# nianticlabs/map-free-reloc

Measured on AMD Instinct MI355X. Metric: image-pairs/sec @ 540x720 (SuperPoint+SuperGlue + PnP w/ depth), higher is better.
Workload: dtype f32 in / f32 accumulate; matrix products of the 3x3 convolutions, attention, the transformer's linear layers and SuperPoint's 1x1 descriptor head on the f16 matrix cores with every fp32 operand carried as TWO f16 terms (xh = rne_f16(x), xl = rne_f16((x - xh) 2^11); weights pre-scaled per output feat

## Files before the change

include/mfr_hip.h:

```cpp
#ifndef MFR_HIP_H
#define MFR_HIP_H
#include <stddef.h>
#include <stdint.h>

#ifdef __cplusplus
extern "C" {
#endif

#define MFR_ABI_VERSION 6

#define MFR_K_F32 0
#define MFR_K_F64 1

#define MFR_E_ARG      (-1)
#define MFR_E_LAUNCH   (-2)
#define MFR_E_WORKSPACE (-3)

#define MFR_ST_OK          0
#define MFR_ST_TOO_FEW     1
#define MFR_ST_BAD_DEPTH   2
#define MFR_ST_NO_MODEL    3
#define MFR_ST_DEGENERATE  4

int mfr_abi_version(void);
// ... 201 lines not shown
                    long long max_record_bytes, float *gray, uint8_t *rgb, int32_t *status, int32_t *rounds, void *workspace,
                    size_t workspace_bytes, int subseq_bits, void *stream);

size_t mfr_png_depth_workspace_bytes(int n, int H, int W);
int mfr_png_depth_decode(const void *headers, const uint8_t *records, const long long *offsets, int n, int H, int W,
                         long long max_record_bytes, void *scratch, size_t scratch_bytes, float *out, int32_t *status, void *stream);

int mfr_resize_gray_bilinear(const uint8_t *rgb, int n, int H, int W, const int32_t *status,
                             const int32_t *y0, const int32_t *y1, const float *fy,
                             const int32_t *x0, const int32_t *x1, const float *fx,
                             int h, int w, float *out, void *stream);

size_t mfr_wino_f16x2_filter_bytes(int Cin, int Cout);
int mfr_wino_f16x2_filter_transform(const float *w, int Cin, int Cout, void *upk, void *stream);
int mfr_conv3x3_wino_f16x2(const float *x, const void *upk, const float *bias, const float *residual, int B, int Cin, int Cout,
                           int H, int W, int act, int pool, float *y, void *stream);
size_t mfr_conv3x3_direct_f16x2_filter_bytes(int Cin, int Cout);
int mfr_conv3x3_direct_f16x2_filter_pack(const float *w, int Cin, int Cout, void *packed, void *stream);
int mfr_conv3x3_direct_f16x2(const float *x, const void *packed, const float *bias, const float *residual, int B, int Cin, int Cout,
                             int H, int W, int act, int pool, float *y, void *stream);
int mfr_conv3x3_direct_f16x2_rows(const float *x, const void *packed, const float *bias, int B, int Cin, int Cout, int H, int W, int act, float *yrows, int ldy, void *stream);
int mfr_conv3x3_direct_f16x2_tiled(const float *x, const void *packed, const float *bias, const float *residual, int B, int Cin, int Cout, int H, int W,
                                   int act, int pool, float *y, int ldrows, int tile_mode, int pitch, void *stream);
int mfr_conv3x3s2_direct_f16x2(const float *x, const void *packed, const float *bias, int B, int Cin, int Cout, int H, int W, int act, float *y, void *stream);
int mfr_sp_conv1ab_f16x2(const float *gray, const float *w1a, const float *b1a, const void *upk1b, const float *bias1b, int B, int H, int W, float *y, void *stream);
size_t mfr_wino_bf16x3_filter_bytes(int Cin, int Cout);
int mfr_wino_bf16x3_filter_transform(const float *w, int Cin, int Cout, void *upk, void *stream);
int mfr_conv3x3_wino_bf16x3(const float *x, const void *upk, const float *bias, const float *residual, int B, int Cin, int Cout,
                            int H, int W, int act, int pool, float *y, void *stream);
size_t mfr_wino_filter_bytes(int Cin, int Cout);
int mfr_wino_filter_transform(const float *w, int Cin, int Cout, float *upk, void *stream);
int mfr_conv3x3_wino(const float *x, const float *upk, const float *bias, const float *residual, int B, int Cin, int Cout,
                     int H, int W, int act, int pool, float *y, void *stream);
int mfr_conv3x3_wino_variant(const float *x, const float *upk, const float *bias, const float *residual, int B, int Cin, int Cout,
                             int H, int W, int act, int pool, int variant, float *y, void *stream);

int mfr_corr_warp_fwd(const float *q, const float *k, const float *v, const float *grid, int B, int Dq, int N,
                      float *warped, float *pos, float *max_score, float *row_max, float *row_sum, void *stream);
int mfr_corr_warp_bwd(const float *q, const float *k, const float *v, const float *grid, int B, int Dq, int N,
                      const float *d_warped, const float *d_pos, const float *d_max, const float *delta,
                      const float *row_max, const float *row_sum, float *dq, float *dk, float *dv, void *stream);

#ifdef __cplusplus
}
#endif
#endif
// ... 1 lines not shown
```

map-free-reloc_amd/_lib.py:

```python
import ctypes as C
import os

_HERE = os.path.dirname(os.path.abspath(__file__))
SO_PATH = os.path.join(_HERE, "csrc", "libmfr_hip.so")

_lib = None

_vp, _i, _d, _u64, _sz = C.c_void_p, C.c_int, C.c_double, C.c_uint64, C.c_size_t

SIGNATURES = {
    "mfr_abi_version": (_i, []),
    "mfr_target_arch": (C.c_char_p, []),
    "mfr_f16x2_guard_bind": (_i, [_vp]),
    "mfr_test_f64_ops": (_i, [_vp, _vp, _vp, _i, _vp, _vp]),
    "mfr_test_sample": (_i, [_u64, _vp, _i, _i, _i, _i, _vp, _vp]),
    "mfr_pnp_workspace_bytes": (_sz, [_i, _i, _i]),
    "mfr_pnp_solve_batch": (_i, [_vp, _vp, _vp, _i, _i, _vp, _i, _i, _vp, _vp, _i, _i, _d, _d, _u64, _vp,
                                 _vp, _sz, _vp, _vp, _vp, _vp, _vp, _vp]),
    "mfr_depth_min": (_i, [_vp, _i, _i, _i, _vp, _vp]),
    "mfr_pnp_lift": (_i, [_vp, _vp, _vp, _i, _i, _vp, _vp, _i, _i, _vp, _i, _vp, _vp, _vp, _vp, _vp]),
    "mfr_pnp_ransac": (_i, [_vp, _vp, _vp, _i, _i, _vp, _i, _i, _d, _d, _u64, _vp, _vp, _vp, _vp, _vp, _vp, _vp,
                            _vp, _vp, _vp, _vp]),
    "mfr_emat_workspace_bytes": (_sz, [_i, _i, _i]),
    "mfr_magsac_lut": (_i, [_vp, _i]),
# ... 41 lines not shown
    "mfr_loftr_coarse_match_variant": (_i, [_vp, _i, _i, _i, _i, _i, C.c_float, C.c_float, _i, _vp, _sz, _vp, _vp, _vp, _vp, _i, _vp]),
    "mfr_loftr_fine_attention": (_i, [_vp, _i, _vp, _vp, _i, _i, _i, _i, _i, _vp, _i, _vp]),
    "mfr_loftr_gather_windows": (_i, [_vp, _i, _i, _i, _i, _vp, _vp, _i, _i, _i, _i, _vp, _vp]),
    "mfr_loftr_fine_match": (_i, [_vp, _vp, _i, _i, _i, _i, C.c_float, _vp, _vp, _vp, _vp, _vp]),
    "mfr_conv3x3_c1_relu": (_i, [_vp, _vp, _vp, _i, _i, _i, _i, _vp, _vp]),
    "mfr_bias_relu_nchw": (_i, [_vp, _vp, _i, _i, _i, _vp]),
    "mfr_conv1x1_nchw": (_i, [_vp, _vp, _vp, _i, _i, _i, _i, _vp, _vp]),
    "mfr_nchw_to_rows": (_i, [_vp, _vp, _i, _i, _i, _i, _vp, C.c_longlong, _i, _vp]),
    "mfr_nchw_to_rows_gather": (_i, [_vp, _vp, _i, _i, _i, _vp, _i, _vp, C.c_longlong, _i, _vp]),
    "mfr_bias_pool2_relu_nchw": (_i, [_vp, _vp, _i, _i, _i, _i, _vp, _vp]),
    "mfr_wino_bf16x3_filter_bytes": (_sz, [_i, _i]),
    "mfr_wino_bf16x3_filter_transform": (_i, [_vp, _i, _i, _vp, _vp]),
    "mfr_conv3x3_wino_bf16x3": (_i, [_vp, _vp, _vp, _vp, _i, _i, _i, _i, _i, _i, _i, _vp, _vp]),
    "mfr_sp_conv1ab_f16x2": (_i, [_vp, _vp, _vp, _vp, _vp, _i, _i, _i, _vp, _vp]),
    "mfr_wino_f16x2_filter_bytes": (_sz, [_i, _i]),
    "mfr_wino_f16x2_filter_transform": (_i, [_vp, _i, _i, _vp, _vp]),
    "mfr_conv3x3_wino_f16x2": (_i, [_vp, _vp, _vp, _vp, _i, _i, _i, _i, _i, _i, _i, _vp, _vp]),
    "mfr_conv3x3_direct_f16x2_filter_bytes": (_sz, [_i, _i]),
    "mfr_conv3x3_direct_f16x2_filter_pack": (_i, [_vp, _i, _i, _vp, _vp]),
    "mfr_conv3x3_direct_f16x2": (_i, [_vp, _vp, _vp, _vp, _i, _i, _i, _i, _i, _i, _i, _vp, _vp]),
    "mfr_conv3x3s2_direct_f16x2": (_i, [_vp, _vp, _vp, _i, _i, _i, _i, _i, _i, _vp, _vp]),
    "mfr_conv3x3_direct_f16x2_rows": (_i, [_vp, _vp, _vp, _i, _i, _i, _i, _i, _i, _vp, _i, _vp]),
    "mfr_conv3x3_direct_f16x2_tiled": (_i, [_vp, _vp, _vp, _vp, _i, _i, _i, _i, _i, _i, _i, _vp, _i, _i, _i, _vp]),
    "mfr_wino_filter_bytes": (_sz, [_i, _i]),
    "mfr_wino_filter_transform": (_i, [_vp, _i, _i, _vp, _vp]),
    "mfr_conv3x3_wino": (_i, [_vp, _vp, _vp, _vp, _i, _i, _i, _i, _i, _i, _i, _vp, _vp]),
    "mfr_conv3x3_wino_variant": (_i, [_vp, _vp, _vp, _vp, _i, _i, _i, _i, _i, _i, _i, _i, _vp, _vp]),
    "mfr_layernorm": (_i, [_vp, _i, _vp, _vp, _vp, _i, C.c_longlong, _i, C.c_float, _vp, _i, _vp]),
    "mfr_conv_gemm_bf16": (_i, [_vp, C.c_longlong, _vp, _vp, C.c_longlong, _vp, _i, _i, _i, _vp, _vp, C.c_longlong, _i,
                                _i, _i, _i, _vp, _vp, _vp, _vp, _vp]),
    "mfr_conv_pack_nhwc_halo": (_i, [_vp, _i, _i, _i, _i, _i, _i, _vp, _i, _vp]),
    "mfr_conv_unpack_nchw": (_i, [_vp, _i, _i, _i, _i, _i, _vp, _vp]),
    "mfr_conv_pack_cm_halo": (_i, [_vp, _i, C.c_longlong, _i, _i, _i, C.c_longlong, _i, _i, C.c_longlong, _vp, _vp]),
    "mfr_upsample2x_add": (_i, [_vp, _vp, _i, _i, _i, _vp]),
    "mfr_upsample_bilinear": (_i, [_vp, _vp, _i, _i, _i, _i, _i, _i, _vp]),
    "mfr_corr_warp_fwd": (_i, [_vp, _vp, _vp, _vp, _i, _i, _i, _vp, _vp, _vp, _vp, _vp, _vp]),
    "mfr_corr_warp_bwd": (_i, [_vp, _vp, _vp, _vp, _i, _i, _i, _vp, _vp, _vp, _vp, _vp, _vp, _vp, _vp, _vp, _vp]),
    "mfr_kabsch_fwd": (_i, [_vp, _i, _vp, _vp]),
    "mfr_kabsch_bwd": (_i, [_vp, _vp, _i, _vp, _vp]),
    "mfr_rootsift": (_i, [_vp, _i, _vp, _vp, _vp]),
    "mfr_desc_ratio_match": (_i, [_vp, _vp, _vp, _vp, _vp, _vp, _i, _i, _i, _vp, _vp, _d, _vp, _vp, _vp, _vp, _i, _vp, _vp]),
    "mfr_sift_workspace_bytes": (_sz, [_i, _i, _i, _i]),
    "mfr_sift_level_offset": (C.c_longlong, [_i, _i, _i, _i, _i, _vp, _vp]),
    "mfr_sift_blur_taps": (_i, [_i, _vp, _vp]),
    "mfr_sift_detect": (_i, [_vp, _i, _i, _i, _i, _i, _i, _vp, _sz, _vp, _vp, _vp, _vp, _vp, _vp, _vp, _vp, _vp]),
    "mfr_jpeg_workspace_bytes": (_sz, [_i, _i, _i, C.c_longlong, _i]),
# ... 57 lines not shown
```

map-free-reloc_amd/csrc/conv_direct.hip:

```cpp
#include <hip/hip_runtime.h>
#include <stdint.h>
#include <type_traits>

#include "../../include/mfr_hip.h"
#include "wave_dev.h"
#include "split_f16.h"
#include "guard.h"

using namespace mfr;

typedef float dc_f32x16 __attribute__((ext_vector_type(16)));
#define DC_OOB 0x80000000u
#define DC_PC 34
#define DC_FRAGS_PER_TAP 6
#ifndef DC_NW
#define DC_NW 4
#endif

#ifdef DC_PROF
__device__ unsigned long long dc_prof[8][64];
#define DC_STAMP(k) do { if (blockIdx.x == (gridDim.x / 2 | 5u) && lane == 0) { __builtin_amdgcn_sched_barrier(0); dc_prof[w][(k)] = __builtin_amdgcn_s_memtime(); __builtin_amdgcn_sched_barrier(0); } } while (0)
extern "C" int *mfr_guard_current(void) { return nullptr; }
#else
#define DC_STAMP(k) do { } while (0)
// ... 28 lines not shown
    if (t >= total) return;
    const int l = (int)(t & 63);
    long long f = t >> 6;
    const int term = (int)(f % 3); f /= 3;
    const int m = (int)(f & 1); f >>= 1;
    const int tap = (int)(f % 9); f /= 9;
    const int c = (int)(f % nks);
    const int cg = (int)(f / nks);
    const int co = cg * 64 + m * 32 + (l & 31);
    const float s = 1.0f / oscale[co];
    unsigned short hw[8];
#pragma unroll
    for (int e = 0; e < 8; ++e) {
        const int ci = 16 * c + 8 * (l >> 5) + e;
        const float v = (co < Cout && ci < Cin) ? w[((size_t)co * Cin + ci) * 9 + tap] * s : 0.f;
        unsigned short wh, wl, wq;
        sf_split_w(v, wh, wl, wq);
        hw[e] = term == 0 ? wh : term == 1 ? wl : wq;
    }
    out[t] = make_uint4((unsigned)hw[0] | ((unsigned)hw[1] << 16), (unsigned)hw[2] | ((unsigned)hw[3] << 16),
                        (unsigned)hw[4] | ((unsigned)hw[5] << 16), (unsigned)hw[6] | ((unsigned)hw[7] << 16));
}

template <int MG, int NW, bool POOL, int STR, int LIN = 0>
__global__ void __launch_bounds__(64 * NW, 8 / NW) conv_direct_f16x2_kernel(
    const float *__restrict__ x, const uint4 *__restrict__ wp, unsigned wp_bytes, const float *__restrict__ oscale, const float *__restrict__ bias,
    const float *__restrict__ residual, float *__restrict__ y, int Cin, int Cout, int H, int W, int nbx, int nby, int S, int ncgw, int nks, int act, int *guard, int ldrows,
    int Pw)
{
    static_assert(STR == 1 || (STR == 2 && !POOL), "stride 1 or 2; no pooled strided variant");
    static_assert(LIN == 0 || (MG == 2 && NW == 4 && !POOL && STR == 1 && LIN % 64 == 0), "linear geometry: MG = 2, stride 1, no pooling");
    using G = DcGeom<MG, NW, STR, LIN>;
    __shared__ __attribute__((aligned(16))) uint4 lds[2 * G::STAGE];
    const int tid = threadIdx.x, lane = tid & 63;
    const int w = __builtin_amdgcn_readfirstlane(tid >> 6);
    const int xcd = blockIdx.x & 7, slot = blockIdx.x >> 3;
    const int cgi = slot % ncgw, s = (slot / ncgw) * 8 + xcd;
    if (s >= S) return;
    const int bx = s % nbx, by = (s / nbx) % nby, b = s / (nbx * nby);
    const int x0 = 32 * bx, y0 = G::TR * by;
    const int u0 = DC_LT * bx;
    const int HW = H * W;
    const int Hout = STR == 1 ? H : (H - 1) / 2 + 1, Wout = STR == 1 ? W : (W - 1) / 2 + 1;
    const bool tail = !POOL && NW == 4 && MG == 2 && cgi == ncgw - 1 && (Cout - cgi * 128 + 31) / 32 == 3;

    const __amdgpu_buffer_rsrc_t rsX = __builtin_amdgcn_make_buffer_rsrc((void *)(x + (size_t)b * Cin * HW), 0, Cin * HW * 4, MFR_RSRC_FLAGS);
    unsigned voff[G::R];
    int wdst[G::R], hh[G::R];
#pragma unroll
    for (int r = 0; r < G::R; ++r) {
        const int h = (G::NT * r + 64 * w) / G::PPAD;
        const int p = G::NT * r + tid - h * G::PPAD;
        if constexpr (LIN > 0) {
            const int il = G::NT * r + tid - (h < 2 ? 0 : 128), hl = (G::NT * r + 64 * w - (h < 2 ? 0 : 128)) / G::PPAD, pl = il - hl * G::PPAD;
            const int U = u0 - Pw - 1 + pl;
            const int yy = (int)((unsigned)max(U, 0) / (unsigned)Pw), xx = max(U, 0) - yy * Pw;
            const bool ok = pl < DC_LT + 2 + 2 * Pw && U >= 0 && yy < H && xx < W;
            voff[r] = ok ? (unsigned)(yy * W + xx) * 4u : DC_OOB;
            hh[r] = hl;
            wdst[r] = il;
            continue;
        }
        const int pr = p / G::PCW, q = p - pr * G::PCW;
        const int pc = STR == 1 ? q : 2 * (q % 33) + q / 33;
        const int gy = STR * y0 - 1 + pr, gx = STR * x0 - 1 + pc;
        const bool ok = h < 2 && p < G::P && pc < STR * 32 + 3 - STR && gy >= 0 && gy < H && gx >= 0 && gx < W;
        voff[r] = ok ? (unsigned)(gy * W + gx) * 4u : DC_OOB;
        hh[r] = h < 2 ? h : 0;
        wdst[r] = h < 2 ? h * G::PPAD + p : G::P + (lane & 15);
    }
    float sv[8];
    auto sload = [&](int r, int c) {
#pragma unroll
        for (int e = 0; e < 8; ++e) {
            const int ch = 16 * c + 8 * hh[r] + e;
            sv[e] = __builtin_bit_cast(float, __builtin_amdgcn_raw_buffer_load_b32(rsX, ch < Cin ? voff[r] : DC_OOB, (unsigned)ch * (unsigned)HW * 4u, 0));
        }
    };
    auto swrite = [&](int r, int buf) {
        unsigned h[4], l[4];
#pragma unroll
        for (int k = 0; k < 4; ++k) sf_split2(sv[2 * k], sv[2 * k + 1], SF_LOW_SCALE, h[k], l[k]);
        lds[buf * G::STAGE + wdst[r]] = make_uint4(h[0], h[1], h[2], h[3]);
        lds[buf * G::STAGE + 2 * G::PPAD + wdst[r]] = make_uint4(l[0], l[1], l[2], l[3]);
    };

    const __amdgpu_buffer_rsrc_t rsW = __builtin_amdgcn_make_buffer_rsrc((void *)wp, 0, (int)wp_bytes, MFR_RSRC_FLAGS);
    const unsigned lane16 = (unsigned)lane * 16u;
// ... 80 lines not shown
                for (int n = 0; n < NB; ++n) acc[m][n] = SF_MFMA(A[m][1], Bh[n], acc[m][n]);
            __builtin_amdgcn_sched_barrier(0);
#pragma unroll
            for (int m = 0; m < MB; ++m) A[m][1] = aload(c, tap + 2, m, 1);
            stage_event(3 * tap + 2);
#pragma unroll
            for (int m = 0; m < MB; ++m)
#pragma unroll
                for (int n = 0; n < NB; ++n) acc[m][n] = SF_MFMA(A[m][0], Bh[n], acc[m][n]);
            __builtin_amdgcn_sched_barrier(0);
        };
        do_tap(DC_IC(0), AE, AO); do_tap(DC_IC(1), AO, AE); do_tap(DC_IC(2), AE, AO); DC_STAMP(4 + 4 * (c & 7)); do_tap(DC_IC(3), AO, AE); do_tap(DC_IC(4), AE, AO);
        do_tap(DC_IC(5), AO, AE); DC_STAMP(5 + 4 * (c & 7)); do_tap(DC_IC(6), AE, AO); do_tap(DC_IC(7), AO, AE); do_tap(DC_IC(8), AE, AO);
#pragma unroll
        for (int m = 0; m < MB; ++m)
#pragma unroll
            for (int t = 0; t < 3; ++t) { const uint4 tmp = AE[m][t]; AE[m][t] = AO[m][t]; AO[m][t] = tmp; }
    }
#undef DC_SL
#undef DC_SW

    const int H = Hout, W = Wout, HW = Hout * Wout;
    DC_STAMP(34);
    auto opix = [&](int n, int lp, int &oy, int &ox) {
        const int u = u0 + 32 * (NB * ng + n) + lp; oy = (int)((unsigned)u / (unsigned)Pw); ox = u - oy * Pw;
    };
    float gchk = 0.f;
    if (guard) {
        bool real[NB];
#pragma unroll
        for (int n = 0; n < NB; ++n) {
            real[n] = true;
            if constexpr (LIN > 0) { int oy, ox; opix(n, lane & 31, oy, ox); real[n] = oy < H && ox < W; }
        }
#pragma unroll
        for (int m = 0; m < MB; ++m)
#pragma unroll
            for (int n = 0; n < NB; ++n)
#pragma unroll
                for (int r = 0; r < 16; ++r) MFR_GUARD_ACC(gchk, LIN > 0 && !real[n] ? 0.f : acc[m][n][r]);
        mfr_guard_commit(guard, gchk);
    }
    const int px0 = x0 + (lane & 31);
    const int half = lane >> 5;
    const int Ho = POOL ? (H >> 1) : H, Wo = POOL ? (W >> 1) : W;
    const size_t cstride = (size_t)Ho * Wo;
    const int cpad1 = (Cout + 63) / 64 * 64 - 1;
    auto activate = [&](float v) { return act == 1 ? fmaxf(v, 0.f) : act == 2 ? (v > 0.f ? v : 0.01f * v) : v; };
    const __amdgpu_buffer_rsrc_t rsY = __builtin_amdgcn_make_buffer_rsrc((void *)(y + (size_t)b * Cout * cstride), 0, (int)(Cout * cstride * 4), MFR_RSRC_FLAGS);
    const __amdgpu_buffer_rsrc_t rsR = __builtin_amdgcn_make_buffer_rsrc((void *)(residual ? residual + (size_t)b * Cout * HW : nullptr), 0, residual ? Cout * HW * 4 : 0, MFR_RSRC_FLAGS);
    if (ldrows > 0) {
        const __amdgpu_buffer_rsrc_t rsQ = __builtin_amdgcn_make_buffer_rsrc((void *)(y + (size_t)b * HW * ldrows), 0, HW * ldrows * 4, MFR_RSRC_FLAGS);
        unsigned pixrow[NB];
#pragma unroll
        for (int n = 0; n < NB; ++n) {
            int oy = y0 + NB * ng + n, px = px0;
            if constexpr (LIN > 0) opix(n, lane & 31, oy, px);
            pixrow[n] = (oy < H && px < W) ? (unsigned)(oy * W + px) * (unsigned)ldrows * 4u : DC_OOB;
        }
        DC_STAMP(36);
#pragma unroll
        for (int m = 0; m < MB; ++m)
#pragma unroll
            for (int q = 0; q < 4; ++q) {
                const int c0 = (mb0 + m) * 32 + 8 * q + 4 * half;
                float o4[4], b4[4];
#pragma unroll
                for (int k = 0; k < 4; ++k) { o4[k] = oscale[min(c0 + k, cpad1)]; b4[k] = bias ? bias[min(c0 + k, Cout - 1)] : 0.f; }
                const unsigned cpart = c0 < Cout ? (unsigned)c0 * 4u : 0x40000000u;
#pragma unroll
                for (int n = 0; n < NB; ++n) {
                    typedef unsigned dc_u32x4 __attribute__((ext_vector_type(4)));
                    const float4 v = make_float4(activate(__builtin_fmaf(acc[m][n][4 * q], o4[0], b4[0])), activate(__builtin_fmaf(acc[m][n][4 * q + 1], o4[1], b4[1])),
                                                 activate(__builtin_fmaf(acc[m][n][4 * q + 2], o4[2], b4[2])), activate(__builtin_fmaf(acc[m][n][4 * q + 3], o4[3], b4[3])));
                    __builtin_amdgcn_raw_buffer_store_b128(__builtin_bit_cast(dc_u32x4, v), rsQ, cpart + pixrow[n], 0, 0);
                }
            }
    } else if (!(W & 3) && (LIN == 0 || !(Pw & 3))) {
        const int L8 = lane >> 3, L7 = lane & 7;
        float os[MB][4], bv[MB][4];
        unsigned cho[MB][4];
#pragma unroll
        for (int m = 0; m < MB; ++m)
#pragma unroll
            for (int j = 0; j < 4; ++j) {
                const int co = (mb0 + m) * 32 + 8 * j + L8;
                os[m][j] = oscale[min(co, cpad1)];
                bv[m][j] = bias ? bias[min(co, Cout - 1)] : 0.f;
                cho[m][j] = co < Cout ? (unsigned)co * (unsigned)cstride * 4u : 0x40000000u;
            }
        unsigned pix[NB];
#pragma unroll
        for (int n = 0; n < NB; ++n) {
            int oy = y0 + NB * ng + n, xg = x0 + 4 * L7;
            if constexpr (LIN > 0) opix(n, 4 * L7, oy, xg);
            if (POOL) pix[n] = ((oy >> 1) < Ho && (xg >> 1) < Wo) ? (unsigned)((oy >> 1) * Wo + (xg >> 1)) * 4u : DC_OOB;
            else      pix[n] = (oy < H && xg < W) ? (unsigned)(oy * W + xg) * 4u : DC_OOB;
        }
        __syncthreads();
        DC_STAMP(36);
        float *tb = (float *)lds + 1024 * w;
        constexpr int NSTEP = POOL ? 2 : 1;
        constexpr int DC_RD = 6;
        float4 rv[POOL ? 1 : MB * NB * 4];
        auto rload = [&](int it) {
            if (!POOL) rv[it] = __builtin_bit_cast(float4, __builtin_amdgcn_raw_buffer_load_b128(rsR, cho[it / (4 * NB)][it & 3] + pix[(it >> 2) % NB], 0, 0));
        };
        if (!POOL && residual) {
#pragma unroll
            for (int it = 0; it < DC_RD; ++it) rload(it);
        }
#pragma unroll
        for (int m = 0; m < MB; ++m)
#pragma unroll
            for (int n = 0; n < NB; n += NSTEP) {
                if (m == 1 && n == 0) DC_STAMP(37);
#pragma unroll
                for (int r = 0; r < 16; ++r)
// ... 13 lines not shown
                            if (it + DC_RD < MB * NB * 4) rload(it + DC_RD);
                            v.x += rv[it].x; v.y += rv[it].y; v.z += rv[it].z; v.w += rv[it].w;
                        }
                        v = make_float4(activate(v.x), activate(v.y), activate(v.z), activate(v.w));
                        typedef unsigned dc_u32x4 __attribute__((ext_vector_type(4)));
                        __builtin_amdgcn_raw_buffer_store_b128(__builtin_bit_cast(dc_u32x4, v), rsY, cho[m][j] + pix[n], 0, 0);
                    }
                }
            }
    } else {
        float osv[MB][16], bvv[MB][16];
#pragma unroll
        for (int m = 0; m < MB; ++m)
#pragma unroll
            for (int r = 0; r < 16; ++r) {
                const int co = (mb0 + m) * 32 + (r & 3) + 8 * (r >> 2) + 4 * half;
                osv[m][r] = oscale[min(co, cpad1)];
                bvv[m][r] = bias ? bias[min(co, Cout - 1)] : 0.f;
            }
        unsigned pixoff[NB];
#pragma unroll
        for (int n = 0; n < NB; ++n) {
            int oy = y0 + NB * ng + n, px = px0;
            if constexpr (LIN > 0) opix(n, lane & 31, oy, px);
            if (POOL) pixoff[n] = (!(lane & 1) && (oy >> 1) < Ho && (px >> 1) < Wo) ? (unsigned)((oy >> 1) * Wo + (px >> 1)) * 4u : DC_OOB;
            else      pixoff[n] = (oy < H && px < W) ? (unsigned)(oy * W + px) * 4u : DC_OOB;
        }
        auto choff = [&](int m, int r) -> unsigned {
            const int co = (mb0 + m) * 32 + (r & 3) + 8 * (r >> 2) + 4 * half;
            return co < Cout ? (unsigned)co * (unsigned)cstride * 4u : 0x40000000u;
        };
        DC_STAMP(36);
        if (POOL) {
#pragma unroll
            for (int m = 0; m < MB; ++m)
#pragma unroll
                for (int r = 0; r < 16; ++r) {
                    const unsigned co4 = choff(m, r);
#pragma unroll
                    for (int n = 0; n < NB; n += 2) {
                        float v = fmaxf(__builtin_fmaf(acc[m][n][r], osv[m][r], bvv[m][r]), __builtin_fmaf(acc[m][n + 1][r], osv[m][r], bvv[m][r]));
                        v = activate(fmaxf(v, __shfl_xor(v, 1)));
                        __builtin_amdgcn_raw_buffer_store_b32(__builtin_bit_cast(unsigned, v), rsY, co4 + pixoff[n], 0, 0);
                    }
                }
        } else {
            constexpr int DC_RD = 4;
// ... 56 lines not shown
int mfr_conv3x3_direct_f16x2_filter_pack(const float *w, int Cin, int Cout, void *packed, void *stream)
{
    if (!w || !packed || Cin <= 0 || Cout <= 0) return MFR_E_ARG;
    const size_t fb = dc_frag_bytes(Cin, Cout);
    const long long total = (long long)(fb / 16);
    float *oscale = (float *)((char *)packed + fb);
    const int cpad = (Cout + 63) / 64 * 64;
    hipLaunchKernelGGL(dc_scale_kernel, dim3((unsigned)cpad), dim3(64), 0, (hipStream_t)stream, w, Cin, Cout, cpad, oscale);
    hipLaunchKernelGGL(dc_pack_kernel, dim3((unsigned)((total + 255) / 256)), dim3(256), 0, (hipStream_t)stream, w, Cin, Cout, (Cin + 15) / 16, total, (const float *)oscale, (uint4 *)packed);
    CHECK_LAUNCH();
    return 0;
}

static bool dc_lin_auto(int W, int Cout, int ldrows)
{
    if (Cout <= 64) return false;
    if (W >= 65 && W <= 80) return true;
    if (W >= 129 && W <= 144) return ldrows == 0;
    return false;
}
#define DC_LIN_AUTO(W, Cout, ldrows) dc_lin_auto(W, Cout, ldrows)
#define DC_LIN_PW_SMALL ((448 - DC_LT - 2) / 2)
#define DC_LIN_PW_LARGE ((576 - DC_LT - 2) / 2)
static int dc_conv(const float *x, const void *packed, const float *bias, const float *residual, int B, int Cin, int Cout, int H, int W,
                   int act, int pool, float *y, int ldrows, int tile_mode, int pitch, void *stream)
{
    if (!x || !packed || !y || B <= 0 || Cin <= 0 || Cout <= 0 || H <= 0 || W <= 0 || act < 0 || act > 2) return MFR_E_ARG;
    if (pool && (H < 2 || W < 2 || residual)) return MFR_E_ARG;
    if ((size_t)4 * (Cin + 15) * H * W >= 0x7fffffffull || (size_t)4 * Cout * H * W >= 0x40000000ull) return MFR_E_ARG;
    const size_t fb = dc_frag_bytes(Cin, Cout);
    if (fb >= 0x7fffffffull) return MFR_E_ARG;
    const int nks = (Cin + 15) / 16;
    const float *oscale = (const float *)((const char *)packed + fb);
    const int mg = Cout > 64 ? 2 : 1;
    const int tr = 4 * DC_NW / mg;
    if (tile_mode < 0 || tile_mode > 2 || pitch < 0) return MFR_E_ARG;
    const bool lin_ok = DC_NW == 4 && mg == 2 && !pool && W + 1 <= DC_LIN_PW_LARGE;
    if (tile_mode == 0) tile_mode = (lin_ok && DC_LIN_AUTO(W, Cout, ldrows)) ? 2 : 1;
    int nbx = (W + 31) / 32, nby = (H + tr - 1) / tr;
    const int ncgw = (Cout + 64 * mg - 1) / (64 * mg);
    if (tile_mode == 2) {
        if (!pitch) pitch = W + 1;
        if (!lin_ok || pitch < W + 1 || pitch > DC_LIN_PW_LARGE) return MFR_E_ARG;
        nbx = (int)(((long long)H * pitch + DC_LT - 1) / DC_LT), nby = 1;
    }
    const long long S = (long long)nbx * nby * B;
    const long long grid = ((S + 7) / 8) * 8 * ncgw;
    if (grid > 0x7fffffffll) return MFR_E_ARG;
    hipStream_t st = (hipStream_t)stream;
    int *guard = mfr_guard_current();
#define DC_LAUNCH(MGV, POOLV, LINV) hipLaunchKernelGGL((conv_direct_f16x2_kernel<MGV, DC_NW, POOLV, 1, LINV>), dim3((unsigned)grid), dim3(64 * DC_NW), 0, st, x, (const uint4 *)packed, (unsigned)fb, oscale, bias, \
                                                        residual, y, Cin, Cout, H, W, nbx, nby, (int)S, ncgw, nks, act, guard, ldrows, pitch)
#if DC_NW == 4
    if (tile_mode == 2) { if (pitch <= DC_LIN_PW_SMALL) DC_LAUNCH(2, false, 448); else DC_LAUNCH(2, false, 576); }
    else
#endif
    if (mg == 1) { if (pool) DC_LAUNCH(1, true, 0); else DC_LAUNCH(1, false, 0); }
    else         { if (pool) DC_LAUNCH(2, true, 0); else DC_LAUNCH(2, false, 0); }
#undef DC_LAUNCH
    CHECK_LAUNCH();
    return 0;
}

int mfr_conv3x3_direct_f16x2(const float *x, const void *packed, const float *bias, const float *residual, int B, int Cin, int Cout, int H, int W,
                             int act, int pool, float *y, void *stream)
{
    return dc_conv(x, packed, bias, residual, B, Cin, Cout, H, W, act, pool, y, 0, 0, 0, stream);
}

int mfr_conv3x3_direct_f16x2_tiled(const float *x, const void *packed, const float *bias, const float *residual, int B, int Cin, int Cout, int H, int W,
                                   int act, int pool, float *y, int ldrows, int tile_mode, int pitch, void *stream)
{
    if (ldrows < 0 || (ldrows > 0 && (ldrows < Cout || (ldrows & 3) || (Cout & 3) || pool || residual || H <= 0 || W <= 0 || (size_t)4 * ldrows * H * W >= 0x40000000ull))) return MFR_E_ARG;
    return dc_conv(x, packed, bias, residual, B, Cin, Cout, H, W, act, pool, y, ldrows, tile_mode, pitch, stream);
}

int mfr_conv3x3_direct_f16x2_rows(const float *x, const void *packed, const float *bias, int B, int Cin, int Cout, int H, int W, int act, float *yrows, int ldy, void *stream)
{
    if (ldy < Cout || (ldy & 3) || (Cout & 3) || H <= 0 || W <= 0 || (size_t)4 * ldy * H * W >= 0x40000000ull) return MFR_E_ARG;
    return dc_conv(x, packed, bias, nullptr, B, Cin, Cout, H, W, act, 0, yrows, ldy, 0, 0, stream);
}

int mfr_conv3x3s2_direct_f16x2(const float *x, const void *packed, const float *bias, int B, int Cin, int Cout, int H, int W, int act, float *y, void *stream)
{
    if (!x || !packed || !y || B <= 0 || Cin <= 0 || Cout <= 0 || H <= 0 || W <= 0 || act < 0 || act > 2) return MFR_E_ARG;
    const int Ho = (H - 1) / 2 + 1, Wo = (W - 1) / 2 + 1;
    if ((size_t)4 * (Cin + 15) * H * W >= 0x7fffffffull || (size_t)4 * Cout * Ho * Wo >= 0x40000000ull) return MFR_E_ARG;
    const size_t fb = dc_frag_bytes(Cin, Cout);
    if (fb >= 0x7fffffffull) return MFR_E_ARG;
    const int nks = (Cin + 15) / 16;
    const float *oscale = (const float *)((const char *)packed + fb);
    const int nbx = (Wo + 31) / 32, nby = (Ho + 3) / 4, ncgw = (Cout + 255) / 256;
    const long long S = (long long)nbx * nby * B;
    const long long grid = ((S + 7) / 8) * 8 * ncgw;
    if (grid > 0x7fffffffll) return MFR_E_ARG;
    hipLaunchKernelGGL((conv_direct_f16x2_kernel<4, 4, false, 2>), dim3((unsigned)grid), dim3(256), 0, (hipStream_t)stream, x, (const uint4 *)packed, (unsigned)fb, oscale, bias,
                       (const float *)nullptr, y, Cin, Cout, H, W, nbx, nby, (int)S, ncgw, nks, act, mfr_guard_current(), 0, 0);
// ... 6 lines not shown
```

map-free-reloc_amd/nets/conv.py:

```python
import torch

from .. import _lib, options

WASTE_LIMIT = {"bf16x3": 0.2, "f16x2": 0.5}


def prefer_split(H, W, split=None):
    mode = options.get("CONV_KERNEL")
    if mode in ("split", "direct"):
        return True
    if mode == "exact":
        return False
    tiles = (W + 1) // 2
    return (-(-tiles // 16) * 16) / tiles - 1.0 <= WASTE_LIMIT[split or options.get("SPLIT")]


class WinoConv3x3:

    def __init__(self, weight, bias, split=None):
        lib = _lib.load(require_gpu=True)
        self.split = split or options.get("SPLIT")
        if self.split not in ("f16x2", "bf16x3"):
            raise ValueError(f"WinoConv3x3: unknown split {self.split!r}")
        self.w, self.b = weight.contiguous(), bias
# ... 28 lines not shown
    def __call__(self, x, act=0, pool=False, residual=None):
        lib = _lib.load()
        mode = options.get("CONV_KERNEL")
        if mode == "direct" or (mode == "auto" and self.split == "f16x2"):
            return self._direct()(x, act=act, pool=pool, residual=residual)
        x = x.contiguous()
        B, C, H, W = x.shape
        y = torch.empty((B, self.co, H // 2, W // 2) if pool else (B, self.co, H, W), dtype=torch.float32, device=x.device)
        res = _lib.ptr(residual.contiguous()) if residual is not None else None
        if self.u_exact is None or prefer_split(H, W, self.split):
            _lib.check(self._conv_split(_lib.ptr(x), _lib.ptr(self.u_split), _lib.ptr(self.b), res, B, C, self.co, H, W, int(act), int(pool),
                                        _lib.ptr(y), _lib.stream_ptr()), f"mfr_conv3x3_wino_{self.split}")
        else:
            _lib.check(lib.mfr_conv3x3_wino(_lib.ptr(x), _lib.ptr(self.u_exact), _lib.ptr(self.b), res, B, C, self.co, H, W, int(act), int(pool),
                                            _lib.ptr(y), _lib.stream_ptr()), "mfr_conv3x3_wino")
        return y


LINEAR_MAX_W = 158


class DirectConv3x3:

    def _tile_mode(self, W, pool):
        tile = options.get("CONV_TILE")
        if tile == "linear":
            return 2 if (self.co > 64 and not pool and W <= LINEAR_MAX_W) else 1
        return 1 if tile == "rows" else 0

    def __init__(self, weight, bias):
        lib = _lib.load(require_gpu=True)
        self.w, self.b = weight.contiguous().float(), bias
        self.co, self.ci = int(weight.shape[0]), int(weight.shape[1])
        self.split = "f16x2"
        self.packed = torch.empty(lib.mfr_conv3x3_direct_f16x2_filter_bytes(self.ci, self.co), dtype=torch.uint8, device=weight.device)
        _lib.check(lib.mfr_conv3x3_direct_f16x2_filter_pack(_lib.ptr(self.w), self.ci, self.co, _lib.ptr(self.packed), _lib.stream_ptr()),
                   "mfr_conv3x3_direct_f16x2_filter_pack")

    def rows(self, x, act=0):
        lib = _lib.load()
        x = x.contiguous()
        B, C, H, W = x.shape
        assert C == self.ci and x.dtype == torch.float32 and self.co % 4 == 0
        y = torch.empty(B, H, W, self.co, dtype=torch.float32, device=x.device)
        mode = self._tile_mode(W, False)
        if mode:
            _lib.check(lib.mfr_conv3x3_direct_f16x2_tiled(_lib.ptr(x), _lib.ptr(self.packed), _lib.ptr(self.b), None, B, C, self.co, H, W, int(act), 0, _lib.ptr(y),
                                                          self.co, mode, 0, _lib.stream_ptr()), "mfr_conv3x3_direct_f16x2_tiled")
            return y
        _lib.check(lib.mfr_conv3x3_direct_f16x2_rows(_lib.ptr(x), _lib.ptr(self.packed), _lib.ptr(self.b), B, C, self.co, H, W, int(act), _lib.ptr(y), self.co,
                                                     _lib.stream_ptr()), "mfr_conv3x3_direct_f16x2_rows")
        return y

    def strided(self, x, act=0):
        lib = _lib.load()
        x = x.contiguous()
        B, C, H, W = x.shape
        assert C == self.ci and x.dtype == torch.float32
        y = torch.empty(B, self.co, (H - 1) // 2 + 1, (W - 1) // 2 + 1, dtype=torch.float32, device=x.device)
        _lib.check(lib.mfr_conv3x3s2_direct_f16x2(_lib.ptr(x), _lib.ptr(self.packed), _lib.ptr(self.b), B, C, self.co, H, W, int(act), _lib.ptr(y), _lib.stream_ptr()),
                   "mfr_conv3x3s2_direct_f16x2")
        return y

    def __call__(self, x, act=0, pool=False, residual=None):
        lib = _lib.load()
        x = x.contiguous()
        B, C, H, W = x.shape
        assert C == self.ci and x.dtype == torch.float32
        y = torch.empty((B, self.co, H // 2, W // 2) if pool else (B, self.co, H, W), dtype=torch.float32, device=x.device)
        res = _lib.ptr(residual.contiguous()) if residual is not None else None
        mode = self._tile_mode(W, pool)
        if mode:
            _lib.check(lib.mfr_conv3x3_direct_f16x2_tiled(_lib.ptr(x), _lib.ptr(self.packed), _lib.ptr(self.b), res, B, C, self.co, H, W, int(act), int(pool),
                                                          _lib.ptr(y), 0, mode, 0, _lib.stream_ptr()), "mfr_conv3x3_direct_f16x2_tiled")
            return y
        _lib.check(lib.mfr_conv3x3_direct_f16x2(_lib.ptr(x), _lib.ptr(self.packed), _lib.ptr(self.b), res, B, C, self.co, H, W, int(act), int(pool),
                                                _lib.ptr(y), _lib.stream_ptr()), "mfr_conv3x3_direct_f16x2")
        return y


class IgemmConv:

    def __init__(self, weight, bias, stride=1, padding=None):
        lib = _lib.load(require_gpu=True)
        co, ci, kh, kw = (int(v) for v in weight.shape)
        self.co, self.ci, self.kh, self.kw = co, ci, kh, kw
        self.stride, self.pad = int(stride), (kh // 2 if padding is None else int(padding))
        K = lib.mfr_conv_igemm_k(ci, kh, kw)
        w = weight.detach().float()
        if ci == 1:
            m = torch.zeros(co, K, dtype=torch.float32, device=w.device)
            m[:, :kh * kw] = w.reshape(co, kh * kw)
        else:
            cpad = K // (kh * kw)
            m = torch.zeros(co, kh * kw, cpad, dtype=torch.float32, device=w.device)
            m[:, :, :ci] = w.permute(0, 2, 3, 1).reshape(co, kh * kw, ci)
            m = m.reshape(co, K)
# ... 25 lines not shown
```

map-free-reloc_amd/options.py:

```python
_SPEC = {
    "SPLIT": ("f16x2", ("f16x2", "bf16x3")),
    "CONV": ("wino", ("wino", "miopen")),
    "CONV_KERNEL": ("auto", ("auto", "split", "exact", "direct")),
    "CONV_TILE": ("auto", ("auto", "rows", "linear")),
    "FUSED_CONV1": (True, (False, True)),
    "FUSED_CONV_RELU": (False, (False, True)),
    "RPR_CONV": ("hip", ("hip", "miopen")),
    "RPR_CONV_BWD": ("lib", ("lib", "hip")),
    "RPR_CONV_ORDER": ("tap_inner", ("tap_inner", "tap_outer")),
    "RPR_WGRAD_SPLITS": (16, None),
    "RPR_ENCODER_NHWC": (False, (False, True)),
}
_VALUES = {k: v[0] for k, v in _SPEC.items()}
_EXPLICIT = set()


def names():
    return sorted(_SPEC)


def default(name):
    return _SPEC[name][0]


def get(name):
    return _VALUES[name]

# ... 54 lines not shown
```

Before: 1352.

## Add band tiling geometry for direct f16x2 3x3 conv with auto selection

Adds a 'band' tile geometry to the direct split-f16 3x3 convolution kernel. Each band of TR output rows is laid out as a padded linear strip of pitch (W+4)&~3, and 32-column blocks are walked along that strip. This cuts the partial-block waste of the 2-D tiling when W is just above a multiple of 32. Auto selection enables it for specific Cout/W ranges, such as W around 257-272 or pooled W around 129-135, when there is no residual or row output. The cost is extra integer division per pixel for address mapping, plus some wasted lanes on padding columns.

```diff
diff --git a/include/mfr_hip.h b/include/mfr_hip.h
--- a/include/mfr_hip.h
+++ b/include/mfr_hip.h
@@ -247,6 +247,13 @@
 int mfr_conv3x3_direct_f16x2_rows(const float *x, const void *packed, const float *bias, int B, int Cin, int Cout, int H, int W, int act, float *yrows, int ldy, void *stream);
 int mfr_conv3x3_direct_f16x2_tiled(const float *x, const void *packed, const float *bias, const float *residual, int B, int Cin, int Cout, int H, int W,
                                    int act, int pool, float *y, int ldrows, int tile_mode, int pitch, void *stream);
+#define MFR_DCONV_AUTO 0
+#define MFR_DCONV_2D 1
+#define MFR_DCONV_LINEAR 2
+#define MFR_DCONV_BAND 3
+int mfr_conv3x3_direct_f16x2_geom(const float *x, const void *packed, const float *bias, const float *residual, int B, int Cin, int Cout, int H, int W,
+                                  int stride, int act, int pool, float *y, int ldrows, int geometry, int pitch, void *stream);
+int mfr_conv3x3_direct_f16x2_auto_geometry(int Cout, int W, int pool, int residual, int ldrows);
 int mfr_conv3x3s2_direct_f16x2(const float *x, const void *packed, const float *bias, int B, int Cin, int Cout, int H, int W, int act, float *y, void *stream);
 int mfr_sp_conv1ab_f16x2(const float *gray, const float *w1a, const float *b1a, const void *upk1b, const float *bias1b, int B, int H, int W, float *y, void *stream);
 size_t mfr_wino_bf16x3_filter_bytes(int Cin, int Cout);
diff --git a/map-free-reloc_amd/_lib.py b/map-free-reloc_amd/_lib.py
--- a/map-free-reloc_amd/_lib.py
+++ b/map-free-reloc_amd/_lib.py
@@ -87,6 +87,8 @@
     "mfr_conv3x3s2_direct_f16x2": (_i, [_vp, _vp, _vp, _i, _i, _i, _i, _i, _i, _vp, _vp]),
     "mfr_conv3x3_direct_f16x2_rows": (_i, [_vp, _vp, _vp, _i, _i, _i, _i, _i, _i, _vp, _i, _vp]),
     "mfr_conv3x3_direct_f16x2_tiled": (_i, [_vp, _vp, _vp, _vp, _i, _i, _i, _i, _i, _i, _i, _vp, _i, _i, _i, _vp]),
+    "mfr_conv3x3_direct_f16x2_geom": (_i, [_vp, _vp, _vp, _vp, _i, _i, _i, _i, _i, _i, _i, _i, _vp, _i, _i, _i, _vp]),
+    "mfr_conv3x3_direct_f16x2_auto_geometry": (_i, [_i, _i, _i, _i, _i]),
     "mfr_wino_filter_bytes": (_sz, [_i, _i]),
     "mfr_wino_filter_transform": (_i, [_vp, _i, _i, _vp, _vp]),
     "mfr_conv3x3_wino": (_i, [_vp, _vp, _vp, _vp, _i, _i, _i, _i, _i, _i, _i, _vp, _vp]),
diff --git a/map-free-reloc_amd/csrc/conv_direct.hip b/map-free-reloc_amd/csrc/conv_direct.hip
--- a/map-free-reloc_amd/csrc/conv_direct.hip
+++ b/map-free-reloc_amd/csrc/conv_direct.hip
@@ -74,7 +74,7 @@
                         (unsigned)hw[4] | ((unsigned)hw[5] << 16), (unsigned)hw[6] | ((unsigned)hw[7] << 16));
 }
 
-template <int MG, int NW, bool POOL, int STR, int LIN = 0>
+template <int MG, int NW, bool POOL, int STR, int LIN = 0, bool BAND = false>
 __global__ void __launch_bounds__(64 * NW, 8 / NW) conv_direct_f16x2_kernel(
     const float *__restrict__ x, const uint4 *__restrict__ wp, unsigned wp_bytes, const float *__restrict__ oscale, const float *__restrict__ bias,
     const float *__restrict__ residual, float *__restrict__ y, int Cin, int Cout, int H, int W, int nbx, int nby, int S, int ncgw, int nks, int act, int *guard, int ldrows,
@@ -82,6 +82,7 @@
 {
     static_assert(STR == 1 || (STR == 2 && !POOL), "stride 1 or 2; no pooled strided variant");
     static_assert(LIN == 0 || (MG == 2 && NW == 4 && !POOL && STR == 1 && LIN % 64 == 0), "linear geometry: MG = 2, stride 1, no pooling");
+    static_assert(!BAND || (STR == 1 && LIN == 0), "band geometry: stride 1; it shares the 2-D tile's staged layout");
     using G = DcGeom<MG, NW, STR, LIN>;
     __shared__ __attribute__((aligned(16))) uint4 lds[2 * G::STAGE];
     const int tid = threadIdx.x, lane = tid & 63;
@@ -92,6 +93,7 @@
     const int bx = s % nbx, by = (s / nbx) % nby, b = s / (nbx * nby);
     const int x0 = 32 * bx, y0 = G::TR * by;
     const int u0 = DC_LT * bx;
+    const int s0 = 32 * bx, nbands = (H + G::TR - 1) / G::TR;
     const int HW = H * W;
     const int Hout = STR == 1 ? H : (H - 1) / 2 + 1, Wout = STR == 1 ? W : (W - 1) / 2 + 1;
     const bool tail = !POOL && NW == 4 && MG == 2 && cgi == ncgw - 1 && (Cout - cgi * 128 + 31) / 32 == 3;
@@ -115,7 +117,12 @@
         }
         const int pr = p / G::PCW, q = p - pr * G::PCW;
         const int pc = STR == 1 ? q : 2 * (q % 33) + q / 33;
-        const int gy = STR * y0 - 1 + pr, gx = STR * x0 - 1 + pc;
+        int gy = STR * y0 - 1 + pr, gx = STR * x0 - 1 + pc;
+        if constexpr (BAND) {
+            const int sc = s0 - 1 + q, k = (int)((unsigned)max(sc, 0) / (unsigned)Pw);
+            gx = sc - k * Pw;
+            gy = k < nbands ? G::TR * k - 1 + pr : H;
+        }
         const bool ok = h < 2 && p < G::P && pc < STR * 32 + 3 - STR && gy >= 0 && gy < H && gx >= 0 && gx < W;
         voff[r] = ok ? (unsigned)(gy * W + gx) * 4u : DC_OOB;
         hh[r] = h < 2 ? h : 0;
@@ -242,8 +249,10 @@
 
     const int H = Hout, W = Wout, HW = Hout * Wout;
     DC_STAMP(34);
+    constexpr bool MAPPED = LIN > 0 || BAND;
     auto opix = [&](int n, int lp, int &oy, int &ox) {
-        const int u = u0 + 32 * (NB * ng + n) + lp; oy = (int)((unsigned)u / (unsigned)Pw); ox = u - oy * Pw;
+        if constexpr (BAND) { const int k = (int)((unsigned)(s0 + lp) / (unsigned)Pw); ox = s0 + lp - k * Pw; oy = G::TR * k + NB * ng + n; }
+        else { const int u = u0 + 32 * (NB * ng + n) + lp; oy = (int)((unsigned)u / (unsigned)Pw); ox = u - oy * Pw; }
     };
     float gchk = 0.f;
     if (guard) {
@@ -251,14 +260,14 @@
 #pragma unroll
         for (int n = 0; n < NB; ++n) {
             real[n] = true;
-            if constexpr (LIN > 0) { int oy, ox; opix(n, lane & 31, oy, ox); real[n] = oy < H && ox < W; }
+            if constexpr (MAPPED) { int oy, ox; opix(n, lane & 31, oy, ox); real[n] = oy < H && ox < W; }
         }
 #pragma unroll
         for (int m = 0; m < MB; ++m)
 #pragma unroll
             for (int n = 0; n < NB; ++n)
 #pragma unroll
-                for (int r = 0; r < 16; ++r) MFR_GUARD_ACC(gchk, LIN > 0 && !real[n] ? 0.f : acc[m][n][r]);
+                for (int r = 0; r < 16; ++r) MFR_GUARD_ACC(gchk, MAPPED && !real[n] ? 0.f : acc[m][n][r]);
         mfr_guard_commit(guard, gchk);
     }
     const int px0 = x0 + (lane & 31);
@@ -275,7 +284,7 @@
 #pragma unroll
         for (int n = 0; n < NB; ++n) {
             int oy = y0 + NB * ng + n, px = px0;
-            if constexpr (LIN > 0) opix(n, lane & 31, oy, px);
+            if constexpr (MAPPED) opix(n, lane & 31, oy, px);
             pixrow[n] = (oy < H && px < W) ? (unsigned)(oy * W + px) * (unsigned)ldrows * 4u : DC_OOB;
         }
         DC_STAMP(36);
@@ -296,7 +305,7 @@
                     __builtin_amdgcn_raw_buffer_store_b128(__builtin_bit_cast(dc_u32x4, v), rsQ, cpart + pixrow[n], 0, 0);
                 }
             }
-    } else if (!(W & 3) && (LIN == 0 || !(Pw & 3))) {
+    } else if (!(W & 3) && (!MAPPED || !(Pw & 3))) {
         const int L8 = lane >> 3, L7 = lane & 7;
         float os[MB][4], bv[MB][4];
         unsigned cho[MB][4];
@@ -313,7 +322,7 @@
 #pragma unroll
         for (int n = 0; n < NB; ++n) {
             int oy = y0 + NB * ng + n, xg = x0 + 4 * L7;
-            if constexpr (LIN > 0) opix(n, 4 * L7, oy, xg);
+            if constexpr (MAPPED) opix(n, 4 * L7, oy, xg);
             if (POOL) pix[n] = ((oy >> 1) < Ho && (xg >> 1) < Wo) ? (unsigned)((oy >> 1) * Wo + (xg >> 1)) * 4u : DC_OOB;
             else      pix[n] = (oy < H && xg < W) ? (unsigned)(oy * W + xg) * 4u : DC_OOB;
         }
@@ -373,7 +382,7 @@
 #pragma unroll
         for (int n = 0; n < NB; ++n) {
             int oy = y0 + NB * ng + n, px = px0;
-            if constexpr (LIN > 0) opix(n, lane & 31, oy, px);
+            if constexpr (MAPPED) opix(n, lane & 31, oy, px);
             if (POOL) pixoff[n] = (!(lane & 1) && (oy >> 1) < Ho && (px >> 1) < Wo) ? (unsigned)((oy >> 1) * Wo + (px >> 1)) * 4u : DC_OOB;
             else      pixoff[n] = (oy < H && px < W) ? (unsigned)(oy * W + px) * 4u : DC_OOB;
         }
@@ -476,6 +485,19 @@
 #define DC_LIN_AUTO(W, Cout, ldrows) dc_lin_auto(W, Cout, ldrows)
 #define DC_LIN_PW_SMALL ((448 - DC_LT - 2) / 2)
 #define DC_LIN_PW_LARGE ((576 - DC_LT - 2) / 2)
+static bool dc_band_auto(int W, int Cout, int pool, bool residual, int ldrows)
+{
+    if (ldrows || residual) return false;
+    if (Cout <= 64) return W >= 257 && W <= 270;
+    if (Cout <= 128) return pool && W >= 129 && W <= 135;
+    return !pool && W >= 257 && W <= 272;
+}
+static bool dc_lin_ok(int W, int Cout, int pool) { return DC_NW == 4 && Cout > 64 && !pool && W + 1 <= DC_LIN_PW_LARGE; }
+static int dc_auto_geometry(int W, int Cout, int pool, bool residual, int ldrows)
+{
+    return (dc_lin_ok(W, Cout, pool) && DC_LIN_AUTO(W, Cout, ldrows)) ? MFR_DCONV_LINEAR : dc_band_auto(W, Cout, pool, residual, ldrows) ? MFR_DCONV_BAND : MFR_DCONV_2D;
+}
+static int dc_band_pitch(int W) { return (W + 4) & ~3; }
 static int dc_conv(const float *x, const void *packed, const float *bias, const float *residual, int B, int Cin, int Cout, int H, int W,
                    int act, int pool, float *y, int ldrows, int tile_mode, int pitch, void *stream)
 {
@@ -488,9 +510,9 @@
     const float *oscale = (const float *)((const char *)packed + fb);
     const int mg = Cout > 64 ? 2 : 1;
     const int tr = 4 * DC_NW / mg;
-    if (tile_mode < 0 || tile_mode > 2 || pitch < 0) return MFR_E_ARG;
-    const bool lin_ok = DC_NW == 4 && mg == 2 && !pool && W + 1 <= DC_LIN_PW_LARGE;
-    if (tile_mode == 0) tile_mode = (lin_ok && DC_LIN_AUTO(W, Cout, ldrows)) ? 2 : 1;
+    if (tile_mode < 0 || tile_mode > 3 || pitch < 0) return MFR_E_ARG;
+    const bool lin_ok = dc_lin_ok(W, Cout, pool);
+    if (tile_mode == 0) tile_mode = dc_auto_geometry(W, Cout, pool, residual != nullptr, ldrows);
     int nbx = (W + 31) / 32, nby = (H + tr - 1) / tr;
     const int ncgw = (Cout + 64 * mg - 1) / (64 * mg);
     if (tile_mode == 2) {
@@ -498,19 +520,28 @@
         if (!lin_ok || pitch < W + 1 || pitch > DC_LIN_PW_LARGE) return MFR_E_ARG;
         nbx = (int)(((long long)H * pitch + DC_LT - 1) / DC_LT), nby = 1;
     }
+    if (tile_mode == 3) {
+        if (!pitch) pitch = dc_band_pitch(W);
+        if (pitch < W + 1 || (pitch & 3) || (long long)nby * pitch > 0x3fffffffll) return MFR_E_ARG;
+        nbx = (int)(((long long)nby * pitch + 31) / 32), nby = 1;
+    }
     const long long S = (long long)nbx * nby * B;
     const long long grid = ((S + 7) / 8) * 8 * ncgw;
     if (grid > 0x7fffffffll) return MFR_E_ARG;
     hipStream_t st = (hipStream_t)stream;
     int *guard = mfr_guard_current();
-#define DC_LAUNCH(MGV, POOLV, LINV) hipLaunchKernelGGL((conv_direct_f16x2_kernel<MGV, DC_NW, POOLV, 1, LINV>), dim3((unsigned)grid), dim3(64 * DC_NW), 0, st, x, (const uint4 *)packed, (unsigned)fb, oscale, bias, \
+#define DC_LAUNCH(MGV, POOLV, LINV, BANDV) hipLaunchKernelGGL((conv_direct_f16x2_kernel<MGV, DC_NW, POOLV, 1, LINV, BANDV>), dim3((unsigned)grid), dim3(64 * DC_NW), 0, st, x, (const uint4 *)packed, (unsigned)fb, oscale, bias, \
                                                         residual, y, Cin, Cout, H, W, nbx, nby, (int)S, ncgw, nks, act, guard, ldrows, pitch)
 #if DC_NW == 4
-    if (tile_mode == 2) { if (pitch <= DC_LIN_PW_SMALL) DC_LAUNCH(2, false, 448); else DC_LAUNCH(2, false, 576); }
+    if (tile_mode == 2) { if (pitch <= DC_LIN_PW_SMALL) DC_LAUNCH(2, false, 448, false); else DC_LAUNCH(2, false, 576, false); }
     else
 #endif
-    if (mg == 1) { if (pool) DC_LAUNCH(1, true, 0); else DC_LAUNCH(1, false, 0); }
-    else         { if (pool) DC_LAUNCH(2, true, 0); else DC_LAUNCH(2, false, 0); }
+    if (tile_mode == 3) {
+        if (mg == 1) { if (pool) DC_LAUNCH(1, true, 0, true); else DC_LAUNCH(1, false, 0, true); }
+        else         { if (pool) DC_LAUNCH(2, true, 0, true); else DC_LAUNCH(2, false, 0, true); }
+    }
+    else if (mg == 1) { if (pool) DC_LAUNCH(1, true, 0, false); else DC_LAUNCH(1, false, 0, false); }
+    else              { if (pool) DC_LAUNCH(2, true, 0, false); else DC_LAUNCH(2, false, 0, false); }
 #undef DC_LAUNCH
     CHECK_LAUNCH();
     return 0;
@@ -525,8 +556,26 @@
 int mfr_conv3x3_direct_f16x2_tiled(const float *x, const void *packed, const float *bias, const float *residual, int B, int Cin, int Cout, int H, int W,
                                    int act, int pool, float *y, int ldrows, int tile_mode, int pitch, void *stream)
 {
+    if (tile_mode > MFR_DCONV_LINEAR) return MFR_E_ARG;
+    return mfr_conv3x3_direct_f16x2_geom(x, packed, bias, residual, B, Cin, Cout, H, W, 1, act, pool, y, ldrows, tile_mode, pitch, stream);
+}
+
+int mfr_conv3x3_direct_f16x2_geom(const float *x, const void *packed, const float *bias, const float *residual, int B, int Cin, int Cout, int H, int W,
+                                  int stride, int act, int pool, float *y, int ldrows, int geometry, int pitch, void *stream)
+{
+    if (stride == 2) {
+        if (geometry < MFR_DCONV_AUTO || geometry > MFR_DCONV_2D || pitch || pool || residual || ldrows) return MFR_E_ARG;
+        return mfr_conv3x3s2_direct_f16x2(x, packed, bias, B, Cin, Cout, H, W, act, y, stream);
+    }
+    if (stride != 1) return MFR_E_ARG;
     if (ldrows < 0 || (ldrows > 0 && (ldrows < Cout || (ldrows & 3) || (Cout & 3) || pool || residual || H <= 0 || W <= 0 || (size_t)4 * ldrows * H * W >= 0x40000000ull))) return MFR_E_ARG;
-    return dc_conv(x, packed, bias, residual, B, Cin, Cout, H, W, act, pool, y, ldrows, tile_mode, pitch, stream);
+    return dc_conv(x, packed, bias, residual, B, Cin, Cout, H, W, act, pool, y, ldrows, geometry, pitch, stream);
+}
+
+int mfr_conv3x3_direct_f16x2_auto_geometry(int Cout, int W, int pool, int residual, int ldrows)
+{
+    if (Cout <= 0 || W <= 0) return MFR_E_ARG;
+    return dc_auto_geometry(W, Cout, pool, residual != 0, ldrows);
 }
 
 int mfr_conv3x3_direct_f16x2_rows(const float *x, const void *packed, const float *bias, int B, int Cin, int Cout, int H, int W, int act, float *yrows, int ldy, void *stream)
diff --git a/map-free-reloc_amd/nets/conv.py b/map-free-reloc_amd/nets/conv.py
--- a/map-free-reloc_amd/nets/conv.py
+++ b/map-free-reloc_amd/nets/conv.py
@@ -74,11 +74,18 @@
 
 class DirectConv3x3:
 
-    def _tile_mode(self, W, pool):
-        tile = options.get("CONV_TILE")
+    def _tile_mode(self, W, pool, rows=False, residual=False):
+        tile, bands = options.get("CONV_TILE"), options.get("CONV_BANDS")
         if tile == "linear":
-            return 2 if (self.co > 64 and not pool and W <= LINEAR_MAX_W) else 1
-        return 1 if tile == "rows" else 0
+            mode = 2 if (self.co > 64 and not pool and W <= LINEAR_MAX_W) else 1
+        else:
+            mode = 1 if tile == "rows" else 0
+        if bands == "auto" or mode == 2:
+            return mode
+        if mode == 0:
+            mode = _lib.load().mfr_conv3x3_direct_f16x2_auto_geometry(self.co, W, int(pool), int(residual), self.co if rows else 0)
+            _lib.check(min(mode, 0), "mfr_conv3x3_direct_f16x2_auto_geometry")
+        return mode if mode == 2 else 3 if bands == "on" else 1
 
     def __init__(self, weight, bias):
         lib = _lib.load(require_gpu=True)
@@ -95,10 +102,10 @@
         B, C, H, W = x.shape
         assert C == self.ci and x.dtype == torch.float32 and self.co % 4 == 0
         y = torch.empty(B, H, W, self.co, dtype=torch.float32, device=x.device)
-        mode = self._tile_mode(W, False)
+        mode = self._tile_mode(W, False, rows=True)
         if mode:
-            _lib.check(lib.mfr_conv3x3_direct_f16x2_tiled(_lib.ptr(x), _lib.ptr(self.packed), _lib.ptr(self.b), None, B, C, self.co, H, W, int(act), 0, _lib.ptr(y),
-                                                          self.co, mode, 0, _lib.stream_ptr()), "mfr_conv3x3_direct_f16x2_tiled")
+            _lib.check(lib.mfr_conv3x3_direct_f16x2_geom(_lib.ptr(x), _lib.ptr(self.packed), _lib.ptr(self.b), None, B, C, self.co, H, W, 1, int(act), 0, _lib.ptr(y),
+                                                         self.co, mode, 0, _lib.stream_ptr()), "mfr_conv3x3_direct_f16x2_geom")
             return y
         _lib.check(lib.mfr_conv3x3_direct_f16x2_rows(_lib.ptr(x), _lib.ptr(self.packed), _lib.ptr(self.b), B, C, self.co, H, W, int(act), _lib.ptr(y), self.co,
                                                      _lib.stream_ptr()), "mfr_conv3x3_direct_f16x2_rows")
@@ -121,10 +128,10 @@
         assert C == self.ci and x.dtype == torch.float32
         y = torch.empty((B, self.co, H // 2, W // 2) if pool else (B, self.co, H, W), dtype=torch.float32, device=x.device)
         res = _lib.ptr(residual.contiguous()) if residual is not None else None
-        mode = self._tile_mode(W, pool)
+        mode = self._tile_mode(W, pool, residual=residual is not None)
         if mode:
-            _lib.check(lib.mfr_conv3x3_direct_f16x2_tiled(_lib.ptr(x), _lib.ptr(self.packed), _lib.ptr(self.b), res, B, C, self.co, H, W, int(act), int(pool),
-                                                          _lib.ptr(y), 0, mode, 0, _lib.stream_ptr()), "mfr_conv3x3_direct_f16x2_tiled")
+            _lib.check(lib.mfr_conv3x3_direct_f16x2_geom(_lib.ptr(x), _lib.ptr(self.packed), _lib.ptr(self.b), res, B, C, self.co, H, W, 1, int(act), int(pool),
+                                                         _lib.ptr(y), 0, mode, 0, _lib.stream_ptr()), "mfr_conv3x3_direct_f16x2_geom")
             return y
         _lib.check(lib.mfr_conv3x3_direct_f16x2(_lib.ptr(x), _lib.ptr(self.packed), _lib.ptr(self.b), res, B, C, self.co, H, W, int(act), int(pool),
                                                 _lib.ptr(y), _lib.stream_ptr()), "mfr_conv3x3_direct_f16x2")
diff --git a/map-free-reloc_amd/options.py b/map-free-reloc_amd/options.py
--- a/map-free-reloc_amd/options.py
+++ b/map-free-reloc_amd/options.py
@@ -3,6 +3,7 @@
     "CONV": ("wino", ("wino", "miopen")),
     "CONV_KERNEL": ("auto", ("auto", "split", "exact", "direct")),
     "CONV_TILE": ("auto", ("auto", "rows", "linear")),
+    "CONV_BANDS": ("auto", ("auto", "on", "off")),
     "FUSED_CONV1": (True, (False, True)),
     "FUSED_CONV_RELU": (False, (False, True)),
     "RPR_CONV": ("hip", ("hip", "miopen")),
```

Result: no change. 1362 (median of 6 runs) (+0.8%).
